# Arbol-Project/dcdf

Measured on NVIDIA B200. Metric: encode_raw_input_GBps, higher is better.
Workload: dtype i64

## Files before the change

### dcdf_b200/csrc/api_encode.cu

```cuda
#include <algorithm>
#include <chrono>
#include <cmath>
#include <cstdlib>
#include <mutex>

#include "encode_big.cuh"
#include "encode_v4.cuh"
#include "encode_v5.cuh"
#include "gather.cuh"
#include "host.hpp"
#include "tree_geo.hpp"
#include "stats.cuh"
#include "xfer.cuh"

using namespace dcdf;

namespace dcdf {
void free_chunk_meta(void* p);
void free_super_meta(void* p);
}

namespace {

int32_t status_from_flags(u32 f, std::string& msg) {
  if (f & EF_NONFINITE) { msg = "cannot convert a non-finite value to fixed point (fixed.rs:39-41)"; return DCDF_ERR_NONFINITE; }
  if (f & EF_OVERFLOW) { msg = "overflow converting to fixed point (fixed.rs:66-69)"; return DCDF_ERR_OVERFLOW; }
  if (f & EF_PRECISION) { msg = "loss of precision converting to fixed point (fixed.rs:51-57)"; return DCDF_ERR_PRECISION_LOSS; }
  if (f & EF_BAD_LEVELS) { msg = "tree levels passed in do not match the levels a nested sub-array needs (superchunk.rs:105-110)"; return DCDF_ERR_BAD_LEVELS; }
  if (f & EF_REGION_EXACT) { msg = "nested region with negatives far below its positive range needs the exact fraction pass, which is not built for nested superchunks yet"; return DCDF_ERR_BAD_ARG; }
  if (f & EF_BAD_FORMAT) { msg = "internal consistency check failed in the encoder"; return DCDF_ERR_BAD_FORMAT; }
  if (f & EF_OUT_CAP) { msg = "output buffer too small"; return DCDF_ERR_BAD_ARG; }
  return DCDF_OK;
}

size_t elem_size(int enc) { return (enc == DCDF_ENC_I32 || enc == DCDF_ENC_F32) ? 4 : 8; }

template <typename Fn>
int32_t guarded(dcdf_ctx* ctx, Fn&& fn) {
  if (!ctx) return DCDF_ERR_BAD_ARG;
  try {
    cudaError_t e = cudaSetDevice(ctx->device);
    if (e != cudaSuccess) throw CudaFail{std::string("cudaSetDevice: ") + cudaGetErrorString(e)};
    fn();
    return DCDF_OK;
  } catch (const ApiFail& f) {
    ctx->last_error = f.msg;
    return f.code;
  } catch (const CudaFail& f) {
    ctx->last_error = f.msg;
    cudaGetLastError();
    return DCDF_ERR_CUDA;
  } catch (const std::bad_alloc&) {
    ctx->last_error = "host out of memory";
    return DCDF_ERR_BAD_ARG;
  } catch (const std::exception& e) {
    ctx->last_error = std::string("unexpected exception: ") + e.what();
    return DCDF_ERR_BAD_ARG;
  } catch (...) {
    ctx->last_error = "unexpected exception";
    return DCDF_ERR_BAD_ARG;
  }
}

void validate_array(const dcdf_array3* a) {
  if (!a || !a->base) api_fail(DCDF_ERR_BAD_ARG, "null array");
  if (a->encoding != DCDF_ENC_I32 && a->encoding != DCDF_ENC_I64 && a->encoding != DCDF_ENC_F32 && a->encoding != DCDF_ENC_F64)
    api_fail(DCDF_ERR_BAD_ARG, "bad encoding %d", a->encoding);
  for (int i = 0; i < 3; i++) {
    if (a->shape[i] <= 0) api_fail(DCDF_ERR_BAD_ARG, "empty array axis %d", i);
  }
  if (a->mem != DCDF_MEM_HOST && a->mem != DCDF_MEM_DEVICE) api_fail(DCDF_ERR_BAD_ARG, "bad mem kind");
}

const void* stage_input(dcdf_ctx* ctx, const dcdf_array3* a) {
  if (a->mem == DCDF_MEM_DEVICE) return a->base;
  int64_t lo = 0, hi = 0;
  for (int i = 0; i < 3; i++) {
    const int64_t ext = (a->shape[i] - 1) * a->strides[i];
    if (ext < 0) lo += ext; else hi += ext;
  }
  const size_t es = elem_size(a->encoding);
  const size_t bytes = (size_t)(hi - lo + 1) * es;
  ctx->input_copy.reserve(bytes);
  static std::mutex upload_mutex[64];
  std::lock_guard<std::mutex> lock(upload_mutex[ctx->device & 63]);
  CK(cudaMemcpyAsync(ctx->input_copy.p, static_cast<const char*>(a->base) + lo * (int64_t)es, bytes, cudaMemcpyHostToDevice, ctx->stream));
  CK(cudaStreamSynchronize(ctx->stream));
  return static_cast<const char*>(ctx->input_copy.p) - lo * (int64_t)es;
}

struct EncodeJob {
  const void* dev_data = nullptr;
  int encoding = 0;
  int64_t strides[3] = {0, 0, 0};
  std::vector<EncUnit> units;
  std::vector<SliceDesc> slices;
  std::vector<uint64_t> table_len;
  uint32_t n_slots = 1;
  uint32_t t_max = 1;
  int plain = 0, req_bits = 0, round = 0, compute_bits = 0;
  int64_t rows = 0, cols = 0;
  size_t input_bytes = 0;
  TreeGeo* tree = nullptr;
};

struct EncodeOut {
  std::vector<EncUnit> units;
  std::vector<UnitResult> results;
  std::vector<uint8_t> stored;
  std::vector<uint64_t> chunk_off;
  std::vector<SliceState> states;
  std::vector<Piece> dac_pieces;
  std::vector<Piece> pieces;
  uint8_t* blob = nullptr;
  uint64_t blob_size = 0;
  uint8_t* dac_blob = nullptr;
  uint64_t dac_blob_size = 0;
  std::vector<uint64_t> dac_off;
  std::vector<NodeState> nstate;
  int64_t* tbl_max = nullptr;
  int64_t* tbl_min = nullptr;
  uint64_t tbl_total = 0;
};

template <typename InT, typename V, bool FULL, int MINB>
void launch_encode_one(dcdf_ctx* ctx, const EncParams& P, u32 grid) {
  const size_t smem = sizeof(EncSmem<V>);
  CK(cudaFuncSetAttribute(k_encode_tiles<InT, V, FULL, MINB>, cudaFuncAttributeMaxDynamicSharedMemorySize, (int)smem));
  k_encode_tiles<InT, V, FULL, MINB><<<grid, ENC_THREADS, smem, FULL ? ctx->stream : ctx->aux_stream>>>(P);
  CK(cudaGetLastError());
  ctx->launches++;
}
template <typename InT, bool FULL>
void launch_encode_v4(dcdf_ctx* ctx, const EncParams& P, u32 grid) {
  constexpr int MINB = 4;
  const u32 stage_limit = std::min<u32>(ctx->opt.stage_limit, (u32)E4_POOL);
  const size_t smem = sizeof(E4Smem);
  CK(cudaFuncSetAttribute(k_encode_v4<InT, MINB, FULL>, cudaFuncAttributeMaxDynamicSharedMemorySize, (int)smem));
  k_encode_v4<InT, MINB, FULL><<<grid, E4_THREADS, smem, FULL ? ctx->stream : ctx->aux_stream>>>(P, stage_limit);
  CK(cudaGetLastError());
  ctx->launches++;
}
template <int G, bool BULK>
void launch_encode_v5_variant(dcdf_ctx* ctx, const EncParams& P, u32 grid) {
  const u32 stage_limit = std::min<u32>(ctx->opt.stage_limit, (u32)E5_POOL);
  const size_t smem = (sizeof(E5Smem) + (BULK ? sizeof(E5Bulk) : 0)) * G;
  CK(cudaFuncSetAttribute(k_encode_v5<G, true, BULK>, cudaFuncAttributeMaxDynamicSharedMemorySize, (int)smem));
  k_encode_v5<G, true, BULK><<<(grid + G - 1) / G, E5_THREADS * G, smem, ctx->stream>>>(P, stage_limit, ctx->opt.fast_sync_mask);
  CK(cudaGetLastError());
  ctx->launches++;
}
template <bool FULL>
void launch_encode_v5(dcdf_ctx* ctx, const EncParams& P, u32 grid) {
  constexpr int G = 6;
  if (FULL && ctx->opt.fast_variant == 1) return launch_encode_v5_variant<4, false>(ctx, P, grid);
  if (FULL && ctx->opt.fast_variant == 2 && ((P.stride_r | P.stride_t) & 3) == 0 && (((uintptr_t)P.data + 4 * 0) & 15) == 0)
    return launch_encode_v5_variant<4, true>(ctx, P, grid);
  const u32 stage_limit = std::min<u32>(ctx->opt.stage_limit, (u32)E5_POOL);
  const size_t smem = sizeof(E5Smem) * G;
  CK(cudaFuncSetAttribute(k_encode_v5<G, FULL>, cudaFuncAttributeMaxDynamicSharedMemorySize, (int)smem));
  k_encode_v5<G, FULL><<<(grid + G - 1) / G, E5_THREADS * G, smem, FULL ? ctx->stream : ctx->aux_stream>>>(P, stage_limit, ctx->opt.fast_sync_mask);
  CK(cudaGetLastError());
  ctx->launches++;
}
void launch_encode_v5_edge(dcdf_ctx* ctx, const EncParams& P, u32 grid) {
  constexpr int G = 12;
  const u32 stage_limit = std::min<u32>(ctx->opt.stage_limit, (u32)E5_POOL_EDGE);
  const size_t smem = sizeof(E5SmemEdge) * G;
  CK(cudaFuncSetAttribute(k_encode_v5_edge<G>, cudaFuncAttributeMaxDynamicSharedMemorySize, (int)smem));
  k_encode_v5_edge<G><<<(grid + G - 1) / G, 32 * G, smem, ctx->aux_stream>>>(P, stage_limit, ctx->opt.fast_sync_mask);
  CK(cudaGetLastError());
  ctx->launches++;
}
template <typename InT>
void launch_encode(dcdf_ctx* ctx, const EncParams& P, u32 grid, int list) {
  if (grid == 0) return;
  if (list >= 5) {
    if (sizeof(InT) == 4) {
      if (list == 5) launch_encode_v5<true>(ctx, P, grid);
      else if (list == 6) launch_encode_v5<false>(ctx, P, grid);
      else launch_encode_v5_edge(ctx, P, grid);
    }
    return;
  }
  const bool force_v2 = ctx->opt.encode_tiles256 != 0;
  if (list == 0 && !force_v2) { launch_encode_v4<InT, true>(ctx, P, grid); return; }
  if (list == 4 && !force_v2) { launch_encode_v4<InT, false>(ctx, P, grid); return; }
  switch (list) {
    case 0: launch_encode_one<InT, int32_t, true, 2>(ctx, P, grid); break;
    case 1: case 4: launch_encode_one<InT, int32_t, false, 2>(ctx, P, grid); break;
    case 2: launch_encode_one<InT, i64, true, 1>(ctx, P, grid); break;
    default: launch_encode_one<InT, i64, false, 1>(ctx, P, grid); break;
  }
}

template <typename InT, bool IS_FLOAT>
void launch_stats(dcdf_ctx* ctx, const StatParams& P) {
  k_unit_stats<InT, IS_FLOAT><<<P.n_units, STAT_THREADS, 0, ctx->stream>>>(P);
  CK(cudaGetLastError());
  ctx->launches++;
}

void time_begin(dcdf_ctx* ctx, int which) { CK(cudaEventRecord(ctx->ev[2 * which], ctx->stream)); }
void time_end(dcdf_ctx* ctx, int which) { CK(cudaEventRecord(ctx->ev[2 * which + 1], ctx->stream)); }
void time_collect(dcdf_ctx* ctx, int which) {
  float ms = 0;
  if (cudaEventElapsedTime(&ms, ctx->ev[2 * which], ctx->ev[2 * which + 1]) == cudaSuccess) ctx->kernel_ms[which] = ms;
  else cudaGetLastError();
}

struct Tracer {
  bool on;
  cudaStream_t st;
  std::chrono::steady_clock::time_point t0;
  Tracer(cudaStream_t s, bool on_) : on(on_), st(s), t0(std::chrono::steady_clock::now()) {}
  void mark(const char* what) {
    if (!on) return;
    cudaStreamSynchronize(st);
    auto t1 = std::chrono::steady_clock::now();
    fprintf(stderr, "[dcdf trace] %-28s %9.3f ms\n", what, std::chrono::duration<double, std::milli>(t1 - t0).count());
    t0 = t1;
  }
};

void run_encode(dcdf_ctx* ctx, EncodeJob& job, EncodeOut& out, bool want_pieces) {
  cudaStream_t st = ctx->stream;
  Tracer tr(st, ctx->opt.trace != 0);
  const u32 n_units = (u32)job.units.size();
  const u32 n_slices = (u32)job.slices.size();
  if (n_units == 0) api_fail(DCDF_ERR_BAD_ARG, "nothing to encode");
  u64 n_pieces = 0;
  for (auto& u : job.units) { u.piece_base = (u32)n_pieces; n_pieces += (u64)u.instants; }
  if (n_pieces > 0xfffffff0ull) api_fail(DCDF_ERR_BAD_ARG, "too many (unit, instant) pairs for one call");
  u64 tbl_total = 0;
  const u32 n_nodes = job.tree ? (u32)job.tree->nodes.size() : 1u;
  const u32 n_tables = n_slices * n_nodes;
  std::vector<uint64_t> table_base(n_tables), table_len(n_tables);
  for (u32 s = 0; s < n_slices; s++) {
    job.slices[s].table_base = tbl_total;
    for (u32 n = 0; n < n_nodes; n++) {
      const u64 off = job.tree ? (u64)job.tree->nodes[n].tbl_off : 0, nch = job.tree ? (u64)job.tree->nodes[n].n_children : 0;
      table_base[(size_t)s * n_nodes + n] = tbl_total + off * (u64)job.slices[s].instants;
      table_len[(size_t)s * n_nodes + n] = job.plain ? 0 : nch * (u64)job.slices[s].instants;
    }
    tbl_total += job.plain ? 0 : job.table_len[s];
  }

  ctx->units.reserve(sizeof(EncUnit) * n_units);
  ctx->ustats.reserve(sizeof(UnitStats) * n_units);
  ctx->istats.reserve(sizeof(InstStats) * (size_t)n_units * job.t_max);
  ctx->slices.reserve(sizeof(SliceDesc) * n_slices + 2 * sizeof(u64) * n_tables);
  ctx->sstate.reserve(sizeof(SliceState) * n_slices);
  ctx->order.reserve(sizeof(u32) * (8 * (size_t)n_units + 8));
  ctx->pieces.reserve(sizeof(Piece) * (n_pieces + 2 * (size_t)n_tables));
  ctx->results.reserve(sizeof(UnitResult) * n_units);
  ctx->stored.reserve(n_units);
  ctx->chunk_off.reserve(sizeof(u64) * ((size_t)n_units + 1));
  ctx->small.reserve(256);
  if (!job.plain) ctx->tbl_scratch.reserve(sizeof(u64) * 4 * tbl_total);
  int64_t *d_tbl_max = nullptr, *d_tbl_min = nullptr;
  if (!job.plain && tbl_total) {
    d_tbl_max = static_cast<int64_t*>(pool_alloc(sizeof(i64) * tbl_total, st));
    d_tbl_min = static_cast<int64_t*>(pool_alloc(sizeof(i64) * tbl_total, st));
  }
  out.tbl_max = d_tbl_max;
  out.tbl_min = d_tbl_min;
  out.tbl_total = tbl_total;

  u32* d_err = ctx->small.as<u32>();
  unsigned long long* d_head = reinterpret_cast<unsigned long long*>(ctx->small.as<u8>() + 8);
  u32* d_counts = reinterpret_cast<u32*>(ctx->small.as<u8>() + 16);

  ctx->pin.reserve(sizeof(EncUnit) * n_units + sizeof(SliceDesc) * n_slices + 2 * sizeof(u64) * n_tables + 64);
  EncUnit* h_units = ctx->pin.as<EncUnit>();
  memcpy(h_units, job.units.data(), sizeof(EncUnit) * n_units);
  SliceDesc* h_slices = reinterpret_cast<SliceDesc*>(h_units + n_units);
  memcpy(h_slices, job.slices.data(), sizeof(SliceDesc) * n_slices);
  u64* h_tb = reinterpret_cast<u64*>(h_slices + n_slices);
  for (u32 i = 0; i < n_tables; i++) { h_tb[i] = table_base[i]; h_tb[n_tables + i] = table_len[i]; }
  copy_by_kernel(ctx, ctx->units.p, h_units, sizeof(EncUnit) * n_units);
  copy_by_kernel(ctx, ctx->slices.p, h_slices, sizeof(SliceDesc) * n_slices + 2 * sizeof(u64) * n_tables);
  const u64* d_table_base = reinterpret_cast<const u64*>(ctx->slices.as<SliceDesc>() + n_slices);
  const u64* d_table_len = d_table_base + n_tables;
  TreeNode* d_nodes = nullptr;
  TreeChild* d_children = nullptr;
  int32_t* d_leaf_unit = nullptr;
  NodeState* d_nstate = nullptr;
  if (job.tree) {
    const TreeGeo& G = *job.tree;
    const size_t b0 = sizeof(TreeNode) * G.nodes.size(), b1 = sizeof(TreeChild) * G.children.size(),
                 b2 = sizeof(int32_t) * G.leaf_unit.size(), b3 = sizeof(NodeState) * (size_t)n_tables;
    ctx->tree_buf.reserve(b0 + b1 + b2 + b3 + 1024);
    u8* tb = ctx->tree_buf.as<u8>();
    d_nodes = reinterpret_cast<TreeNode*>(tb);
    d_children = reinterpret_cast<TreeChild*>(tb + ((b0 + 255) & ~size_t(255)));
    d_leaf_unit = reinterpret_cast<int32_t*>(reinterpret_cast<u8*>(d_children) + ((b1 + 255) & ~size_t(255)));
    d_nstate = reinterpret_cast<NodeState*>(reinterpret_cast<u8*>(d_leaf_unit) + ((b2 + 255) & ~size_t(255)));
    upload_small(ctx, d_nodes, G.nodes.data(), b0);
    upload_small(ctx, d_children, G.children.data(), b1);
    upload_small(ctx, d_leaf_unit, G.leaf_unit.data(), b2);
  }

  tr.mark("scratch + uploads");
  StatParams SP;
  SP.data = job.dev_data;
  SP.stride_t = job.strides[0]; SP.stride_r = job.strides[1]; SP.stride_c = job.strides[2];
  SP.units = ctx->units.as<EncUnit>();
  SP.n_units = n_units;
  SP.t_max = job.t_max;
  SP.ustats = ctx->ustats.as<UnitStats>();
  SP.istats = ctx->istats.as<InstStats>();
  time_begin(ctx, KT_STATS);
  switch (job.encoding) {
    case DCDF_ENC_F32: launch_stats<float, true>(ctx, SP); break;
    case DCDF_ENC_F64: launch_stats<double, true>(ctx, SP); break;
    case DCDF_ENC_I32: launch_stats<int32_t, false>(ctx, SP); break;
    default: launch_stats<i64, false>(ctx, SP); break;
  }
  time_end(ctx, KT_STATS);
  tr.mark("k_unit_stats");

  FinalizeParams FP;
  FP.slices = ctx->slices.as<SliceDesc>();
  FP.state = ctx->sstate.as<SliceState>();
  FP.units_in = ctx->units.as<EncUnit>();
  FP.units = ctx->units.as<EncUnit>();
  FP.ustats = SP.ustats;
  FP.istats = SP.istats;
  FP.t_max = job.t_max;
  FP.n_slots = job.n_slots;
  FP.encoding = job.encoding;
  FP.req_bits = job.req_bits; FP.round = job.round; FP.compute_bits = job.compute_bits; FP.plain = job.plain;
  FP.tbl_min = d_tbl_min; FP.tbl_max = d_tbl_max;
  FP.order = ctx->order.as<u32>();
  FP.order_pitch = n_units;
  FP.order_counts = d_counts;
  FP.stored = ctx->stored.as<u8>();
  FP.err = d_err;
  CK(cudaMemsetAsync(ctx->small.p, 0, 64, st));
  k_finalize_phase1<<<n_slices, 256, 0, st>>>(FP, n_slices);
  CK(cudaGetLastError());
  ctx->launches++;
  const bool is_float = job.encoding == DCDF_ENC_F32 || job.encoding == DCDF_ENC_F64;
  if (is_float && job.compute_bits) {
    SliceState* ss = ctx->sstate.as<SliceState>();
    std::vector<SliceState> hs(n_slices);
    read_small(ctx, hs.data(), ss, sizeof(SliceState) * n_slices);
    sync_reads(ctx);
    bool any = false;
    for (auto& s : hs) any = any || s.need_exact;
    if (any) {
      ctx->exact.reserve((sizeof(i64) + 5 * sizeof(int)) * n_slices + 64);
      std::vector<i64> t0(n_slices);
      std::vector<int> inst(n_slices);
      for (u32 s = 0; s < n_slices; s++) { t0[s] = job.slices[s].t0; inst[s] = job.slices[s].instants; }
      i64* d_t0 = ctx->exact.as<i64>();
      int* d_inst = reinterpret_cast<int*>(d_t0 + n_slices);
      upload_small(ctx, d_t0, t0.data(), sizeof(i64) * n_slices);
      upload_small(ctx, d_inst, inst.data(), sizeof(int) * n_slices);
      ExactParams XP;
      XP.data = job.dev_data;
      XP.stride_t = job.strides[0]; XP.stride_r = job.strides[1]; XP.stride_c = job.strides[2];
      XP.rows = job.rows; XP.cols = job.cols;
      XP.slice_t0 = d_t0; XP.slice_instants = d_inst;
      std::vector<int> need(n_slices), maxfb(n_slices);
      for (u32 s = 0; s < n_slices; s++) { need[s] = hs[s].need_exact; maxfb[s] = hs[s].maxfb; }
      int* d_need = d_inst + n_slices;
      int* d_maxfb = d_need + n_slices;
      int* d_f = d_maxfb + n_slices;
      int* d_round = d_f + n_slices;
      upload_small(ctx, d_need, need.data(), sizeof(int) * n_slices);
      upload_small(ctx, d_maxfb, maxfb.data(), sizeof(int) * n_slices);
      CK(cudaMemsetAsync(d_f, 0, 2 * sizeof(int) * n_slices, st));
      XP.slice_need = d_need; XP.slice_maxfb = d_maxfb; XP.slice_f = d_f; XP.slice_round = d_round;
      dim3 grid((unsigned)std::min<int64_t>(4 * ctx->sm_count, 65535), n_slices);
      if (job.encoding == DCDF_ENC_F32) k_fraction_exact<float><<<grid, 256, 0, st>>>(XP, n_slices);
      else k_fraction_exact<double><<<grid, 256, 0, st>>>(XP, n_slices);
      CK(cudaGetLastError());
      ctx->launches++;
      std::vector<int> f(n_slices), r(n_slices);
      read_small(ctx, f.data(), d_f, sizeof(int) * n_slices);
      read_small(ctx, r.data(), d_round, sizeof(int) * n_slices);
      sync_reads(ctx);
      for (u32 s = 0; s < n_slices; s++) { hs[s].f_exact = f[s]; hs[s].round_exact = r[s]; }
      upload_small(ctx, ss, hs.data(), sizeof(SliceState) * n_slices);
    }
  }
  if (job.tree) {
    const TreeGeo& G = *job.tree;
    TreeParams TP;
    TP.slices = FP.slices; TP.state = FP.state;
    TP.nodes = d_nodes; TP.children = d_children; TP.n_nodes = n_nodes;
    TP.leaf_unit = d_leaf_unit; TP.leaf_cols = G.leaf_cols; TP.leaf_side = G.leaf_side;
    TP.tbl_per_instant = G.tbl_per_instant;
    TP.nstate = d_nstate;
    TP.units = ctx->units.as<EncUnit>();
    TP.ustats = SP.ustats; TP.istats = SP.istats; TP.t_max = job.t_max;
    TP.encoding = job.encoding; TP.round = job.round; TP.req_bits = job.req_bits;
    TP.allow_fast = job.encoding == DCDF_ENC_F32 && !ctx->opt.no_fast_encode && job.strides[2] == 1;
    TP.tbl_min = d_tbl_min; TP.tbl_max = d_tbl_max;
    TP.order = FP.order; TP.order_pitch = FP.order_pitch; TP.order_counts = FP.order_counts;
    TP.stored = FP.stored; TP.err = d_err;
    k_finalize_tree<<<n_slices, 256, 0, st>>>(TP, n_slices);
  } else {
    k_finalize_phase2<<<n_slices, 256, 0, st>>>(FP, n_slices);
  }
  CK(cudaGetLastError());
  ctx->launches++;

  tr.mark("finalize");
  if (ctx->arena_hint == 0) ctx->arena_hint = std::max<size_t>(job.input_bytes / 2 + (8u << 20), 16u << 20);
  std::vector<uint8_t> head_buf(64);
  u32 sticky = 0;
  for (int attempt = 0;; attempt++) {
    ctx->arena.reserve(ctx->arena_hint);
    const u64 arena_cap = ctx->arena.cap;
    CK(cudaMemsetAsync(d_head, 0, 8, st));
    EncParams EP;
    EP.data = job.dev_data;
    EP.stride_t = job.strides[0]; EP.stride_r = job.strides[1]; EP.stride_c = job.strides[2];
    EP.units = ctx->units.as<EncUnit>();
    EP.pieces = ctx->pieces.as<Piece>();
    EP.results = ctx->results.as<UnitResult>();
    EP.arena = ctx->arena.as<u8>();
    EP.arena_cap = arena_cap;
    EP.arena_head = d_head;
    EP.err = d_err;
    time_begin(ctx, KT_ENCODE);
    CK(cudaEventRecord(ctx->fork_ev, st));
    CK(cudaStreamWaitEvent(ctx->aux_stream, ctx->fork_ev, 0));
    for (int list = 7; list >= 0; list--) {
      EP.order = FP.order + (size_t)list * n_units;
      EP.order_count = d_counts + list;
      switch (job.encoding) {
        case DCDF_ENC_F32: launch_encode<float>(ctx, EP, n_units, list); break;
        case DCDF_ENC_F64: launch_encode<double>(ctx, EP, n_units, list); break;
        case DCDF_ENC_I32: launch_encode<int32_t>(ctx, EP, n_units, list); break;
        default: launch_encode<i64>(ctx, EP, n_units, list); break;
      }
    }
    CK(cudaEventRecord(ctx->join_ev, ctx->aux_stream));
    CK(cudaStreamWaitEvent(st, ctx->join_ev, 0));
    time_end(ctx, KT_ENCODE);
    tr.mark("k_encode_tiles");
    if (!job.plain) {
      TableDacParams TP;
      TP.tbl_min = d_tbl_min; TP.tbl_max = d_tbl_max;
      TP.table_base = d_table_base; TP.table_len = d_table_len;
      TP.alive = reinterpret_cast<const int*>(d_nstate);
      TP.scratch = ctx->tbl_scratch.as<u64>();
      TP.total = tbl_total;
      TP.pieces = ctx->pieces.as<Piece>() + n_pieces;
      TP.arena = ctx->arena.as<u8>(); TP.arena_cap = arena_cap; TP.arena_head = d_head; TP.err = d_err;
      k_table_dac<<<dim3(n_tables, 2), ENC_THREADS, 0, st>>>(TP);
      CK(cudaGetLastError());
      ctx->launches++;
    }
    tr.mark("k_table_dac");
    k_scan_units<<<1, 1024, 0, st>>>(ctx->results.as<UnitResult>(), ctx->stored.as<u8>(), n_units, ctx->chunk_off.as<u64>());
    CK(cudaGetLastError());
    ctx->launches++;
    read_small(ctx, head_buf.data(), ctx->small.p, 64);
    sync_reads(ctx);
    u32 flags;
    u64 head;
    memcpy(&flags, head_buf.data(), 4);
    memcpy(&head, head_buf.data() + 8, 8);
    memcpy(ctx->last_list_counts, head_buf.data() + 16, sizeof ctx->last_list_counts);
    sticky |= flags & ~(u32)EF_ARENA_FULL;
    std::string msg;
    if ((flags & EF_ARENA_FULL) && status_from_flags(sticky, msg) == DCDF_OK) {
      if (attempt >= 3) api_fail(DCDF_ERR_CUDA, "arena overflow persisted after growth");
      ctx->arena_hint = (size_t)head + (size_t)head / 16 + (1u << 20);
      CK(cudaMemsetAsync(d_err, 0, 4, st));
      continue;
    }
    flags = sticky;
    int32_t code = status_from_flags(flags, msg);
    if (code != DCDF_OK) {
      pool_free(d_tbl_max);
      pool_free(d_tbl_min);
      out.tbl_max = out.tbl_min = nullptr;
      throw ApiFail{code, msg};
    }
    break;
  }
  time_collect(ctx, KT_STATS);
  time_collect(ctx, KT_ENCODE);
  tr.mark("scan + flags readback");

  out.units.resize(n_units);
  out.results.resize(n_units);
  out.stored.resize(n_units);
  out.chunk_off.resize((size_t)n_units + 1);
  out.states.resize(n_slices);
  read_small(ctx, out.units.data(), ctx->units.p, sizeof(EncUnit) * n_units);
  read_small(ctx, out.results.data(), ctx->results.p, sizeof(UnitResult) * n_units);
  read_small(ctx, out.stored.data(), ctx->stored.p, n_units);
  read_small(ctx, out.chunk_off.data(), ctx->chunk_off.p, sizeof(u64) * ((size_t)n_units + 1));
  read_small(ctx, out.states.data(), ctx->sstate.p, sizeof(SliceState) * n_slices);
  if (!job.plain) {
    out.dac_pieces.resize(2 * (size_t)n_tables);
    read_small(ctx, out.dac_pieces.data(), ctx->pieces.as<Piece>() + n_pieces, sizeof(Piece) * 2 * n_tables);
    out.nstate.resize(n_tables);
    read_small(ctx, out.nstate.data(), d_nstate, sizeof(NodeState) * n_tables);
  }
  if (want_pieces) {
    out.pieces.resize(n_pieces);
    CK(cudaMemcpyAsync(out.pieces.data(), ctx->pieces.p, sizeof(Piece) * n_pieces, cudaMemcpyDeviceToHost, st));
  }
  sync_reads(ctx);

  tr.mark("tables readback");
  out.blob_size = out.chunk_off[n_units];
  out.blob = static_cast<uint8_t*>(pool_alloc(out.blob_size + 64, st));
  CK(cudaMemsetAsync(out.blob + out.blob_size, 0, 64, st));
  GatherParams GP;
  GP.units = ctx->units.as<EncUnit>();
  GP.results = ctx->results.as<UnitResult>();
  GP.stored = ctx->stored.as<u8>();
  GP.pieces = ctx->pieces.as<Piece>();
  GP.chunk_off = ctx->chunk_off.as<u64>();
  GP.arena = ctx->arena.as<u8>();
  GP.out = out.blob;
  GP.out_cap = out.blob_size;
  GP.encoding = job.encoding;
  GP.n_units = n_units;
  GP.err = d_err;
  tr.mark("blob alloc");
  time_begin(ctx, KT_GATHER);
  k_gather_chunks<<<n_units, 256, 0, st>>>(GP);
  CK(cudaGetLastError());
  ctx->launches++;
  if (!job.plain) {
    out.dac_off.resize(2 * (size_t)n_tables);
    u64 off = 0;
    for (u32 i = 0; i < 2 * n_tables; i++) { out.dac_off[i] = off; off += out.dac_pieces[i].size; }
    out.dac_blob_size = off;
    out.dac_blob = static_cast<uint8_t*>(pool_alloc(off + 16, st));
    ctx->query_aux.reserve(sizeof(u64) * 2 * n_tables);
    upload_small(ctx, ctx->query_aux.p, out.dac_off.data(), sizeof(u64) * 2 * n_tables);
    GatherDacParams DP;
    DP.pieces = ctx->pieces.as<Piece>() + n_pieces;
    DP.dst_off = ctx->query_aux.as<u64>();
    DP.arena = ctx->arena.as<u8>();
    DP.out = out.dac_blob;
    k_gather_dacs<<<2 * n_tables, 256, 0, st>>>(DP);
    CK(cudaGetLastError());
    ctx->launches++;
  }
  time_end(ctx, KT_GATHER);
  read_small(ctx, head_buf.data(), ctx->small.p, 4);
  sync_reads(ctx);
  time_collect(ctx, KT_GATHER);
  tr.mark("gather");
  u32 flags;
  memcpy(&flags, head_buf.data(), 4);
  flags |= sticky;
  std::string msg;
  int32_t code = status_from_flags(flags, msg);
  if (code != DCDF_OK) throw ApiFail{code, msg};
}


struct BigResult {
  uint8_t* blob = nullptr;
  uint64_t size = 0;
  uint32_t snapshots = 0, logs = 0;
  std::vector<uint32_t> block_instants;
};

struct BigScratch {
  dcdf_ctx* ctx;
  u8* base = nullptr;
  size_t used = 0, cap = 0;
  template <typename T>
  T* take(size_t n) {
    used = (used + 255) & ~size_t(255);
    T* p = reinterpret_cast<T*>(base + used);
    used += n * sizeof(T);
    return p;
  }
};

unsigned big_grid(dcdf_ctx* ctx, u64 n, int block = 256) {
  return (unsigned)std::max<u64>(1, std::min<u64>((n + block - 1) / block, (u64)ctx->sm_count * 16));
}

void big_scan(dcdf_ctx* ctx, const u64* in, u64 n, u64* out, u64* block_sums) {
  if (n == 0) return;
  const unsigned nb = (unsigned)((n + SCAN_ITEMS - 1) / SCAN_ITEMS);
// ... 828 lines not shown
```

### dcdf_b200/csrc/encode_v5.cuh

```cuda
#pragma once
#include <type_traits>

#include "encode_v4.cuh"

namespace dcdf {

constexpr int E5_THREADS = 64;
constexpr int E5_POOL = 9 * 1024;
constexpr int E5_POOL_EDGE = 5 * 1024;

template <int TT, int POOL>
struct E5SmemT {
  __align__(16) u8 pool[POOL + 16];
  int4 cell[16][TT];
  int2 l4s[4][TT];
  int2 l4t[4][TT];
  u32 leaf[16][TT];
  u32 qx[4][TT];
  u32 qn[4][TT];
  int4 rec1[4];
  int2 ent1[4];
  u32 wt[2][2][4];
  u32 bm_off[12], bm_len[12];
  u32 n_bm;
// ... 101 lines not shown
    if (t.len > 3) b3[p3] = (u8)(t.z >> 24);
  }
}
template <bool FULL>
DCDF_DEVINL void e5_load_node(const float* pn, i64 sr, uint4 (&raw)[4], int rl, int cl, int vec) {
#pragma unroll
  for (int r = 0; r < 4; r++) {
    if (FULL || (r < rl && cl >= 4)) {
      const float* pr = pn + (i64)r * sr;
      if (vec == 2) {
        asm volatile("ld.shared.v4.u32 {%0, %1, %2, %3}, [%4];" : "=r"(raw[r].x), "=r"(raw[r].y), "=r"(raw[r].z), "=r"(raw[r].w)
                     : "r"((u32)__cvta_generic_to_shared(pr)));
      } else if (vec) {
        raw[r] = __ldg(reinterpret_cast<const uint4*>(pr));
      } else {
        raw[r] = make_uint4(__float_as_uint(__ldg(pr)), __float_as_uint(__ldg(pr + 1)), __float_as_uint(__ldg(pr + 2)), __float_as_uint(__ldg(pr + 3)));
      }
    } else {
      raw[r] = make_uint4(0, 0, 0, 0);
      if (r < rl) {
        const float* pr = pn + (i64)r * sr;
        if (cl > 0) raw[r].x = __float_as_uint(__ldg(pr));
        if (cl > 1) raw[r].y = __float_as_uint(__ldg(pr + 1));
        if (cl > 2) raw[r].z = __float_as_uint(__ldg(pr + 2));
      }
    }
  }
}
DCDF_DEVINL int e5_conv_raw(float x, float scale2) { return __float_as_int(__fmaf_rn(x, scale2, 12582912.0f)) - (0x4B400000 - 1); }
DCDF_DEVINL int e5_nan0(u32 bits, int f) { return (bits & 0x7fffffffu) > 0x7f800000u ? 0 : f; }
template <bool FULL>
DCDF_DEVINL void e5_quads(const uint4 (&raw)[4], float scale2, int4 (&q)[4], int rl, int cl) {
#pragma unroll
  for (int h = 0; h < 2; h++) {
    const uint4 u = raw[2 * h], l = raw[2 * h + 1];
    q[2 * h] = make_int4(e5_conv_raw(__uint_as_float(u.x), scale2), e5_conv_raw(__uint_as_float(u.y), scale2),
                         e5_conv_raw(__uint_as_float(l.x), scale2), e5_conv_raw(__uint_as_float(l.y), scale2));
    q[2 * h + 1] = make_int4(e5_conv_raw(__uint_as_float(u.z), scale2), e5_conv_raw(__uint_as_float(u.w), scale2),
                             e5_conv_raw(__uint_as_float(l.z), scale2), e5_conv_raw(__uint_as_float(l.w), scale2));
  }
  {
    const int m01 = max(max(max(q[0].x, q[0].y), max(q[0].z, q[0].w)), max(max(q[1].x, q[1].y), max(q[1].z, q[1].w)));
    const int m23 = max(max(max(q[2].x, q[2].y), max(q[2].z, q[2].w)), max(max(q[3].x, q[3].y), max(q[3].z, q[3].w)));
    if (max(m01, m23) > (1 << 28)) {
#pragma unroll
      for (int h = 0; h < 2; h++) {
        const uint4 u = raw[2 * h], l = raw[2 * h + 1];
        q[2 * h] = make_int4(e5_nan0(u.x, q[2 * h].x), e5_nan0(u.y, q[2 * h].y), e5_nan0(l.x, q[2 * h].z), e5_nan0(l.y, q[2 * h].w));
        q[2 * h + 1] = make_int4(e5_nan0(u.z, q[2 * h + 1].x), e5_nan0(u.w, q[2 * h + 1].y), e5_nan0(l.z, q[2 * h + 1].z), e5_nan0(l.w, q[2 * h + 1].w));
      }
    }
  }
#pragma unroll
  for (int h = 0; h < 2; h++) {
    if (!FULL) {
      const bool ru = 2 * h < rl, rw = 2 * h + 1 < rl;
      if (!(ru && cl > 0)) q[2 * h].x = E4_NONE;
      if (!(ru && cl > 1)) q[2 * h].y = E4_NONE;
      if (!(rw && cl > 0)) q[2 * h].z = E4_NONE;
      if (!(rw && cl > 1)) q[2 * h].w = E4_NONE;
      if (!(ru && cl > 2)) q[2 * h + 1].x = E4_NONE;
      if (!(ru && cl > 3)) q[2 * h + 1].y = E4_NONE;
      if (!(rw && cl > 2)) q[2 * h + 1].z = E4_NONE;
      if (!(rw && cl > 3)) q[2 * h + 1].w = E4_NONE;
    }
  }
}
DCDF_DEVINL const float* e5_node_ptr(const float* pt, i64 sr, int a) { return pt + (i64)(4 * (a >> 1)) * sr + 4 * (a & 1); }
template <bool FULL>
DCDF_DEVINL int e5_dx(int a, int b) { return e4_sub(e4_o0<FULL>(a), e4_o0<FULL>(b)); }
DCDF_DEVINL int e5_dn(int a, int b) { return e4_sub(a, b); }

DCDF_DEVINL u32 e5_low4(int a, int b, int c, int d) { return __byte_perm(__byte_perm((u32)a, (u32)b, 0x0040), __byte_perm((u32)c, (u32)d, 0x0040), 0x5410); }
DCDF_DEVINL u32 e5_zz4(u32 p) { return ((p + p) & 0xfefefefeu) ^ (((p >> 7) & 0x01010101u) * 0xffu); }
DCDF_DEVINL u32 e5_pack4(u32 z0, u32 z1, u32 z2, u32 z3) { return (z0 & 0xffu) | ((z1 & 0xffu) << 8) | ((z2 & 0xffu) << 16) | (z3 << 24); }
template <bool ALIGNED = false>
DCDF_DEVINL void e5_store_word(u8* p, u32 w) {
  if (ALIGNED || (((uintptr_t)p) & 3u) == 0) *reinterpret_cast<u32*>(p) = w;
  else { p[0] = (u8)w; p[1] = (u8)(w >> 8); p[2] = (u8)(w >> 16); p[3] = (u8)(w >> 24); }
}

template <bool FULL, int TT = E5_THREADS>
__device__ __noinline__ void e5_long_node(bool as_snapshot, const float* pn, i64 sr, float scale2, const int4* scell, int2 n4, u32 in5a,
                                          u8* xb1, u8* nb1, u32* pos , int rl, int cl, int vec) {
  int4 q[4];
  if (!as_snapshot) {
    uint4 raw[4];
    e5_load_node<FULL>(pn, sr, raw, rl, cl, vec);
    e5_quads<FULL>(raw, scale2, q, rl, cl);
  }
  u32 lx1 = pos[0], rx1 = pos[1], rn1 = pos[2];
  u32 zx[4], zn[4];
#pragma unroll
  for (int b = 0; b < 4; b++) {
    const int4 s = scell[b * TT];
    const int4 t = as_snapshot ? s : q[b];
    int qmax, qmin, sqmax, sqmin;
    e4_qmm<FULL>(t, qmax, qmin);
    e4_qmm<FULL>(s, sqmax, sqmin);
    zx[b] = zigzag32(as_snapshot ? e5_dx<FULL>(n4.x, qmax) : e5_dx<FULL>(qmax, sqmax));
    zn[b] = zigzag32(as_snapshot ? e5_dn(qmin, n4.y) : e5_dn(qmin, sqmin));
    if ((in5a >> (3 - b)) & 1u) {
      const u32 z0 = zigzag32(as_snapshot ? e5_dx<FULL>(qmax, t.x) : e4_sub(t.x, s.x)), z1 = zigzag32(as_snapshot ? e5_dx<FULL>(qmax, t.y) : e4_sub(t.y, s.y));
      const u32 z2 = zigzag32(as_snapshot ? e5_dx<FULL>(qmax, t.z) : e4_sub(t.z, s.z)), z3 = zigzag32(as_snapshot ? e5_dx<FULL>(qmax, t.w) : e4_sub(t.w, s.w));
      if (z0 > 0xffu) xb1[lx1++] = (u8)(z0 >> 8);
      if (z1 > 0xffu) xb1[lx1++] = (u8)(z1 >> 8);
      if (z2 > 0xffu) xb1[lx1++] = (u8)(z2 >> 8);
      if (z3 > 0xffu) xb1[lx1++] = (u8)(z3 >> 8);
    }
  }
#pragma unroll
  for (int b = 0; b < 4; b++)
    if (zx[b] > 0xffu) xb1[rx1++] = (u8)(zx[b] >> 8);
#pragma unroll
  for (int b = 0; b < 4; b++)
    if (((in5a >> (3 - b)) & 1u) && zn[b] > 0xffu) nb1[rn1++] = (u8)(zn[b] >> 8);
  pos[0] = lx1; pos[1] = rx1; pos[2] = rn1;
}

DCDF_DEVINL u32 e5_smem_u32(const void* p) { return (u32)__cvta_generic_to_shared(p); }
DCDF_DEVINL void e5_mbar_init(unsigned long long* b, u32 count) {
  asm volatile("mbarrier.init.shared::cta.b64 [%0], %1;" ::"r"(e5_smem_u32(b)), "r"(count) : "memory");
}
DCDF_DEVINL void e5_mbar_expect_tx(unsigned long long* b, u32 bytes) {
  asm volatile("mbarrier.arrive.expect_tx.shared::cta.b64 _, [%0], %1;" ::"r"(e5_smem_u32(b)), "r"(bytes) : "memory");
}
DCDF_DEVINL void e5_mbar_wait(unsigned long long* b, u32 parity) {
  asm volatile(
      "{\n\t.reg .pred P1;\n\t"
      "E5_WAIT:\n\t"
      "mbarrier.try_wait.parity.shared::cta.b64 P1, [%0], %1;\n\t"
      "@P1 bra E5_DONE;\n\t"
      "bra E5_WAIT;\n\t"
      "E5_DONE:\n\t}" ::"r"(e5_smem_u32(b)), "r"(parity) : "memory");
}
DCDF_DEVINL void e5_bulk_g2s(void* smem, const void* g, u32 bytes, unsigned long long* b) {
  asm volatile("cp.async.bulk.shared::cluster.global.mbarrier::complete_tx::bytes [%0], [%1], %2, [%3];" ::"r"(e5_smem_u32(smem)),
               "l"(g), "r"(bytes), "r"(e5_smem_u32(b))
               : "memory");
}
struct E5Bulk {
  __align__(16) float raw[64 * 64];
  __align__(8) unsigned long long mbar;
  unsigned long long pad_;
};

template <int NW>
DCDF_DEVINL void e5_tile_sync(int slot) {
  if (NW == 1) __syncwarp();
  else asm volatile("bar.sync %0, 64;" ::"r"(slot + 1) : "memory");
}

template <int G, bool FULL, bool BULK, int NW = 2>
DCDF_DEVINL void e5_body(const EncParams& P, const u32 stage_limit, const int sync_mask);
template <int G, bool FULL, bool BULK = false>
__global__ void __launch_bounds__(E5_THREADS * G, 1) k_encode_v5(const EncParams P, const u32 stage_limit, const int sync_mask) {
  e5_body<G, FULL, BULK>(P, stage_limit, sync_mask);
}
template <int G>
__global__ void __launch_bounds__(32 * G, 1) k_encode_v5_edge(const EncParams P, const u32 stage_limit, const int sync_mask) {
  e5_body<G, false, false, 1>(P, stage_limit, sync_mask);
}
template <int G, bool FULL, bool BULK, int NW>
DCDF_DEVINL void e5_body(const EncParams& P, const u32 stage_limit, const int sync_mask) {
  static_assert(NW == 2 || (NW == 1 && !FULL && !BULK), "one-warp tiles are clipped edge tiles");
  constexpr int TT = 32 * NW;
  using Smem = std::conditional_t<NW == 2, E5Smem, E5SmemEdge>;
  const int vec = BULK ? 2 : (((P.stride_r | P.stride_t) & 3) == 0 && (((uintptr_t)P.data) & 15) == 0) ? 1 : 0;
  extern __shared__ __align__(16) unsigned char smem_raw[];
  const int slot = threadIdx.x / TT;
  constexpr size_t kSlab = sizeof(Smem) + (BULK ? sizeof(E5Bulk) : 0);
  Smem& S = *reinterpret_cast<Smem*>(smem_raw + (size_t)slot * kSlab);
  E5Bulk& SB = *reinterpret_cast<E5Bulk*>(smem_raw + (size_t)slot * kSlab + sizeof(Smem));

  const u32 n_order = *P.order_count;
  if (blockIdx.x * (u32)G >= n_order) return;
  const u32 order_idx = blockIdx.x * (u32)G + (u32)slot;
  const bool tile_live = order_idx < n_order;
  const u32 unit_idx = P.order[tile_live ? order_idx : blockIdx.x * (u32)G];
  EncUnit unit = P.units[unit_idx];
  if (!tile_live) unit.instants = 0;
  int max_instants = 0;
  for (int g = 0; g < G; g++) {
    const u32 oi = blockIdx.x * (u32)G + (u32)g;
    if (oi < n_order) max_instants = max(max_instants, P.units[P.order[oi]].instants);
  }
  const int tid = threadIdx.x % TT, lane = tid & 31, warp = tid >> 5;
  const int node = NW == 2 ? tid : unit.rows <= 32 ? lane : lane < 16 ? lane : lane + 16;
  const float scale2 = (float)((i64)2 << unit.bits);
  const i64 sr = BULK ? 64 : P.stride_r;
  const float* const base = BULK ? SB.raw + (8 * (int)morton_row(tid)) * 64 + 8 * (int)morton_col(tid)
                                 : static_cast<const float*>(P.data) + unit.base + (i64)(8 * (int)morton_row(node)) * sr + 8 * (int)morton_col(node);
  const float* const my_row = static_cast<const float*>(P.data) + unit.base + (i64)tid * P.stride_r;
  auto fetch_instant = [&](int t) {
    if (tid == 0) e5_mbar_expect_tx(&SB.mbar, 64u * 256u);
    e5_bulk_g2s(SB.raw + 64 * tid, my_row + (i64)t * P.stride_t, 256u, &SB.mbar);
  };
  if (BULK) {
    if (tid == 0) {
      e5_mbar_init(&SB.mbar, 1u);
      asm volatile("fence.mbarrier_init.release.cluster;" ::: "memory");
    }
    e5_tile_sync<NW>(slot);
    if (unit.instants > 0) fetch_instant(0);
  }
  const bool owner2 = (lane & 3) == 0;
  const bool is1 = (u32)(lane - 1) < 4u;
  const int k1 = node >> 4;
  const int rl8 = unit.rows - 8 * (int)morton_row(node), cl8 = unit.cols - 8 * (int)morton_col(node);
#define E5_RL(a) (rl8 - 4 * ((a) >> 1))
#define E5_CL(a) (cl8 - 4 * ((a) & 1))

  {
    uint4* z = reinterpret_cast<uint4*>(S.pool);
    for (int i = tid; i < (int)(sizeof(S.pool) / 16); i += TT) z[i] = make_uint4(0, 0, 0, 0);
  }
  if (!FULL) {
    for (int q = 0; q < 16; q++) S.cell[q][tid] = make_int4(E4_NONE, E4_NONE, E4_NONE, E4_NONE);
    for (int a = 0; a < 4; a++) S.l4s[a][tid] = make_int2(E4_NONE, INT32_MAX);
  }
  if (NW == 1 && lane == 0) {
    const u32 missing1 = unit.rows <= 32 ? 0xcu : 0xau;
    for (int k = 0; k < 4; k++) {
      if ((missing1 >> k) & 1u) {
        S.rec1[k] = make_int4(E4_NONE, INT32_MAX, 0, 1);
        S.ent1[k] = make_int2(0, 0);
      }
    }
    for (int c = 0; c < 2; c++)
      for (int i = 0; i < 4; i++) S.wt[1][c][i] = 0u;
  }

  u32 err = 0;
  int s3max = 0, s3min = 0, s2max = 0, s2min = 0, s1max = 0, s1min = 0, s0max = 0, s0min = 0;
  u32 n_logs = 0, n_snap = 0, n_log_total = 0;
  u64 total_bytes = 0;

#pragma unroll 1
  for (int inst = 0; inst < max_instants; inst++) {
    if ((inst & sync_mask) == 0) __syncthreads();
    if (inst >= unit.instants) continue;
    const bool first = inst == 0;
    const float* const pt = BULK ? base : base + (i64)inst * P.stride_t;
    if (BULK) e5_mbar_wait(&SB.mbar, (u32)inst & 1u);
    if (!BULK && inst + 1 < unit.instants) {
#pragma unroll
      for (int r = 0; r < 8; r++)
        if (FULL || (r < rl8 && cl8 > 0)) asm volatile("prefetch.global.L2 [%0];" ::"l"(pt + P.stride_t + (i64)r * sr));
    }
    const bool forced = first || n_logs == 254u;

    u32 u5 = 0, eq5 = 0, u4 = 0, eq4 = 0;
    E5Cand L, C;
    L.ml = 0; L.mq = 0; L.mu = 0; L.in5 = 0; L.in4 = 0; L.in3 = L.in2 = L.in1 = false;
    C.ml = 0; C.mq = 0; C.mu = 0; C.in5 = 0; C.in4 = 0; C.in3 = C.in2 = C.in1 = false;
    int t3max = 0, t3min = 0, diff3 = 0;
    bool eq3 = false, u3 = false;
    int t2max = 0, t2min = 0, t1max = 0, t1min = 0, t0max = 0, t0min = 0;
    bool u2 = false, eq2 = false, u0 = false, eq0 = false;
    int n1max = 0, n1min = 0, l_e1max = 0, l_e1min = 0;
    bool n1un = false, n1eq = false;
    u32 l_in1 = 0, s_in1 = 0;
    bool l_in0 = false, s_in0 = false;
    u32 wl[4] = {0, 0, 0, 0}, ws[4] = {0, 0, 0, 0};
    E5Tot T;
    u32 ntop = 0, item_cnt = 0, item_size = 0;
    bool as_snapshot = forced;
    u32 my_size = 0, log_size = 0;

#pragma unroll 1
    for (int pass = forced ? 1 : 0; pass < 2; pass++) {
      t3max = INT32_MIN; t3min = INT32_MAX;
      u5 = 0; u4 = 0;
      uint4 raw[4];
      e5_load_node<FULL>(e5_node_ptr(pt, sr, 0), sr, raw, E5_RL(0), E5_CL(0), vec);
      if (pass == 0) {
        eq3 = true;
#pragma unroll 1
        for (int a = 0; a < 4; a++) {
          int4 q[4];
          e5_quads<FULL>(raw, scale2, q, E5_RL(a), E5_CL(a));
          if (a < 3) e5_load_node<FULL>(e5_node_ptr(pt, sr, a + 1), sr, raw, E5_RL(a + 1), E5_CL(a + 1), vec);
          const int2 s4 = S.l4s[a][tid];
          int amax = INT32_MIN, amin = INT32_MAX, dfirst = 0;
          bool aeq = true;
          u32 leaf16 = 0, u5n = 0, e5n = 0, qx = 0, qn = 0;
          u32 exw = 0, enw = 0;
          u32 ovx = 0, ovn = 0, ovm = 0;
#pragma unroll
          for (int b = 0; b < 4; b++) {
            const int4 t = q[b], sq = S.cell[4 * a + b][tid];
            int qmax, qmin, sqmax, sqmin;
            e4_qmm<FULL>(t, qmax, qmin);
            e4_qmm<FULL>(sq, sqmax, sqmin);
            const int d0 = e4_sub(t.x, sq.x), d1 = e4_sub(t.y, sq.y), d2 = e4_sub(t.z, sq.z), d3 = e4_sub(t.w, sq.w);
            const int ex = e5_dx<FULL>(qmax, sqmax), en = e5_dn(qmin, sqmin);
            const bool e5 = (((d1 ^ d0) | (d2 ^ d0) | (d3 ^ d0)) == 0);
            if (e4_unif<FULL>(qmax, qmin)) u5n |= 1u << (3 - b);
            if (e5) e5n |= 1u << (3 - b);
            u32 leafw = e5_zz4(e5_low4(d0, d1, d2, d3));
            exw = __byte_perm(exw, (u32)ex, b == 0 ? 0x3214 : b == 1 ? 0x3240 : b == 2 ? 0x3410 : 0x4210);
            enw = __byte_perm(enw, (u32)en, b == 0 ? 0x3214 : b == 1 ? 0x3240 : b == 2 ? 0x3410 : 0x4210);
            if ((((u32)d0 + 128u) | ((u32)d1 + 128u) | ((u32)d2 + 128u) | ((u32)d3 + 128u) | ((u32)ex + 128u) | ((u32)en + 128u)) > 255u) {
              if (e4_longer<1>(d0)) leaf16 |= 1u << (15 - 4 * b);
              if (e4_longer<1>(d1)) leaf16 |= 1u << (14 - 4 * b);
              if (e4_longer<1>(d2)) leaf16 |= 1u << (13 - 4 * b);
              if (e4_longer<1>(d3)) leaf16 |= 1u << (12 - 4 * b);
              if (e4_longer<1>(ex)) qx |= 1u << (3 - b);
              if (e4_longer<1>(en)) qn |= 1u << (3 - b);
              if ((((u32)d0 + 32768u) | ((u32)d1 + 32768u) | ((u32)d2 + 32768u) | ((u32)d3 + 32768u)) > 65535u) err |= EF_BAD_FORMAT;
              leafw = e5_pack4(zigzag32(d0), zigzag32(d1), zigzag32(d2), zigzag32(d3));
              ovx |= (zigzag32(ex) & 0xffu) << (8 * b);
              ovn |= (zigzag32(en) & 0xffu) << (8 * b);
              ovm |= 0xffu << (8 * b);
            }
            S.leaf[4 * a + b][tid] = leafw;
            amax = max(amax, qmax); amin = min(amin, qmin);
            if (b == 0) dfirst = d0;
            aeq = aeq && e5 && d0 == dfirst;
          }
          const u32 zxw = (e5_zz4(exw) & ~ovm) | ovx, znw = (e5_zz4(enw) & ~ovm) | ovn;
          S.qx[a][tid] = zxw;
          S.qn[a][tid] = znw;
          S.l4t[a][tid] = make_int2(amax, amin);
          L.ml |= (u64)leaf16 << (48 - 16 * a);
          L.mq |= (qx << (12 - 4 * a)) | (qn << (28 - 4 * a));
          u5 |= u5n << (12 - 4 * a);
          eq5 |= e5n << (12 - 4 * a);
          if (e4_unif<FULL>(amax, amin)) u4 |= 1u << (3 - a);
          if (aeq) eq4 |= 1u << (3 - a);
          if (e4_longer<1>(e5_dx<FULL>(amax, s4.x))) L.mu |= 1u << (3 - a);
          if (e4_longer<1>(e5_dn(amin, s4.y))) L.mu |= 1u << (7 - a);
          t3max = max(t3max, amax); t3min = min(t3min, amin);
          if (a == 0) diff3 = dfirst;
          eq3 = eq3 && aeq && dfirst == diff3;
        }
        if (e4_longer<1>(e5_dx<FULL>(t3max, s3max))) L.mu |= 1u << 8;
// ... 369 lines not shown
      }
    }
    if (emit) {
      if (x4) {
        u32 rx1 = bx4 + e4_f4(pre[1]), rn1 = bn4 + e4_f4(pre[3]);
        u32 zx[4], zn[4];
#pragma unroll
        for (int a = 0; a < 4; a++) {
          const int2 n4 = S.l4t[a][tid];
          const int2 s4 = as_snapshot ? make_int2(0, 0) : S.l4s[a][tid];
          zx[a] = zigzag32(as_snapshot ? e5_dx<FULL>(t3max, n4.x) : e5_dx<FULL>(n4.x, s4.x));
          zn[a] = zigzag32(as_snapshot ? e5_dn(n4.y, t3min) : e5_dn(n4.y, s4.y));
        }
        e5_store_word<decltype(in_shared)::value>(xb0 + Pn4 + 4u * R3, e5_pack4(zx[0], zx[1], zx[2], zx[3]));
        u8* dmn = nb0 + Mn4 + R4;
        if (W.mu & 0xffu) {
#pragma unroll
          for (int a = 0; a < 4; a++)
            if (zx[a] > 0xffu) rx1 = e5_hi(xb1, zx[a], rx1);
        }
#pragma unroll
        for (int a = 0; a < 4; a++) {
          if ((W.in4 >> (3 - a)) & 1u) {
            *dmn++ = (u8)zn[a];
            if (zn[a] > 0xffu) rn1 = e5_hi(nb1, zn[a], rn1);
          }
        }
      }
      if (x3) {
        const u32 zx = zigzag32(as_snapshot ? e5_dx<FULL>(t2max, t3max) : e5_dx<FULL>(t3max, s3max));
        xb0[Pn3 + 4u * R2p + (u32)(node & 3)] = (u8)zx;
        if (zx > 0xffu) e5_hi(xb1, zx, bx3 + e4_f3(pre[1]));
        if (W.in3) {
          const u32 zn = zigzag32(as_snapshot ? e5_dn(t3min, t2min) : e5_dn(t3min, s3min));
          nb0[Mn3 + R3] = (u8)zn;
          if (zn > 0xffu) e5_hi(nb1, zn, bn3 + e4_f3(pre[3]));
        }
      }
      if (x2 && owner2) {
        const u32 zx = zigzag32(as_snapshot ? e5_dx<FULL>(t1max, t2max) : e5_dx<FULL>(t2max, s2max));
        xb0[Pn2 + 4u * R1 + (u32)((node >> 2) & 3)] = (u8)zx;
        if (zx > 0xffu) e5_hi(xb1, zx, bx2 + e4_f2(pre[1]));
        if (W.in2) {
          const u32 zn = zigzag32(as_snapshot ? e5_dn(t2min, t1min) : e5_dn(t2min, s2min));
          nb0[Mn2 + R2own] = (u8)zn;
          if (zn > 0xffu) e5_hi(nb1, zn, bn2 + e4_f2(pre[3]));
        }
      }
#pragma unroll
      for (int r = 0; r < NTOP; r++) {
        const bool mx = NW == 2 ? warp == 0 : r == 0;
        if (top[r].len > 0) (mx ? xb0 : nb0)[top[r].pos0] = (u8)top[r].z;
        if (top[r].len > 1) (mx ? xb1 : nb1)[top[r].pos1] = (u8)(top[r].z >> 8);
        if (__any_sync(0xffffffffu, top[r].len > 2)) e5_top_long(true, out, top[r], mx ? 2 : 6, item_hdr, item_cnt, item_at);
      }
      if ((NW == 1 || warp == 1) && lane >= 16) {
        const u32 i = lane - 16u;
        if (i < 13u) {
          const u32 word = i < 5u ? (u32)unit.rows : i < 9u ? (u32)unit.cols : 64u;
          out[i] = i == 0 ? (u8)2 : (u8)(word >> (8u * ((12u - i) & 3u)));
        } else if (i == 13u) {
          out[x_hdr0 - 1] = (u8)x_levels;
        } else if (i == 14u) {
          out[n_hdr0 - 1] = (u8)n_levels;
        }
      }
    }
    e5_tile_sync<NW>(slot);
    if (BULK && inst + 1 < unit.instants) fetch_instant(inst + 1);

    if (emit) {
      const u32 n_fix = as_snapshot ? 1u : 2u;
      const u32 n_bm = n_fix + x_levels + n_levels;
#pragma unroll 1
      for (u32 i = warp; i < n_bm; i += NW) {
        const int src = (int)(i < n_fix ? i : i < n_fix + x_levels ? 2u + (i - n_fix) : 6u + (i - n_fix - x_levels));
        const u32 hdr = shfl(item_hdr, src), len = shfl(item_cnt, src);
        if (lane == 0) {
          store_be32(out + hdr, len);
          store_be32(out + hdr + 4, 4u);
        }
        const u32 blocks = len >> 7;
        u8* const index = out + hdr + 8u;
        const u8* const words = index + 4u * blocks;
        u32 carry = 0;
#pragma unroll 1
        for (u32 b0 = 0; b0 < blocks; b0 += 32u) {
          const u32 b = b0 + lane;
          u32 c = b < blocks ? e4_popc_bytes16(words + 16u * b) : 0u;
#pragma unroll
          for (int d = 1; d < 32; d <<= 1) {
            const u32 n = __shfl_up_sync(0xffffffffu, c, d);
            if (lane >= d) c += n;
          }
          if (b < blocks) e4_store_be32(index + 4u * b, carry + c);
          carry += shfl(c, 31);
        }
      }
    }
    if (decltype(in_shared)::value && tid == 0) publish_piece();
    e5_tile_sync<NW>(slot);

    if constexpr (decltype(in_shared)::value) {
      piece_off = S.piece_off;
      fits = piece_off + (((u64)my_size + 15ull) & ~15ull) <= P.arena_cap;
      if (!fits) err |= EF_ARENA_FULL;
      u32* src = reinterpret_cast<u32*>(S.pool);
      uint4* dst = reinterpret_cast<uint4*>(P.arena + piece_off);
      const u32 sh = 8u * shift;
      const u32 n16 = (my_size + 15u) / 16u;
#pragma unroll 1
      for (u32 i = tid; i < n16; i += TT) {
        const uint4 v = *reinterpret_cast<const uint4*>(src + 4u * i);
        const u32 nx = src[4u * i + 4u];
        uint4 o;
        o.x = __funnelshift_r(v.x, v.y, sh); o.y = __funnelshift_r(v.y, v.z, sh);
        o.z = __funnelshift_r(v.z, v.w, sh); o.w = __funnelshift_r(v.w, nx, sh);
        if (fits) dst[i] = o;
      }
      e5_tile_sync<NW>(slot);
#pragma unroll 1
      for (u32 i = tid; i < n16 + 1u; i += TT) *reinterpret_cast<uint4*>(src + 4u * i) = make_uint4(0, 0, 0, 0);
    }

    };
    if (staged) emission(std::true_type{});
    else emission(std::false_type{});

    if (as_snapshot) {
      s3max = t3max; s3min = t3min; s2max = t2max; s2min = t2min; s1max = t1max; s1min = t1min; s0max = t0max; s0min = t0min;
      n_snap++;
      n_logs = 0;
      total_bytes += 1;
    } else {
      n_logs++;
      n_log_total++;
    }
    total_bytes += my_size;
  }

  if (tid == 0 && tile_live) {
    UnitResult r;
    r.bytes = total_bytes + 6;
    r.snapshots = n_snap;
    r.logs = n_log_total;
    P.results[unit_idx] = r;
  }
  err = __reduce_or_sync(0xffffffffu, err);
  if (lane == 0 && err) atomicOr(P.err, err);
#undef E5_RL
#undef E5_CL
}

}
```

Baseline: 663.1.

## Merge full and edge tile encoders into one persistent work-stealing kernel

After: 654.3 (median of 6 runs). 0.987x the previous value.

```diff
diff --git a/dcdf_b200/csrc/api_encode.cu b/dcdf_b200/csrc/api_encode.cu
--- a/dcdf_b200/csrc/api_encode.cu
+++ b/dcdf_b200/csrc/api_encode.cu
@@ -153,9 +153,6 @@
 template <bool FULL>
 void launch_encode_v5(dcdf_ctx* ctx, const EncParams& P, u32 grid) {
   constexpr int G = 6;
-  if (FULL && ctx->opt.fast_variant == 1) return launch_encode_v5_variant<4, false>(ctx, P, grid);
-  if (FULL && ctx->opt.fast_variant == 2 && ((P.stride_r | P.stride_t) & 3) == 0 && (((uintptr_t)P.data + 4 * 0) & 15) == 0)
-    return launch_encode_v5_variant<4, true>(ctx, P, grid);
   const u32 stage_limit = std::min<u32>(ctx->opt.stage_limit, (u32)E5_POOL);
   const size_t smem = sizeof(E5Smem) * G;
   CK(cudaFuncSetAttribute(k_encode_v5<G, FULL>, cudaFuncAttributeMaxDynamicSharedMemorySize, (int)smem));
@@ -163,23 +160,29 @@
   CK(cudaGetLastError());
   ctx->launches++;
 }
-void launch_encode_v5_edge(dcdf_ctx* ctx, const EncParams& P, u32 grid) {
-  constexpr int G = 12;
-  const u32 stage_limit = std::min<u32>(ctx->opt.stage_limit, (u32)E5_POOL_EDGE);
-  const size_t smem = sizeof(E5SmemEdge) * G;
-  CK(cudaFuncSetAttribute(k_encode_v5_edge<G>, cudaFuncAttributeMaxDynamicSharedMemorySize, (int)smem));
-  k_encode_v5_edge<G><<<(grid + G - 1) / G, 32 * G, smem, ctx->aux_stream>>>(P, stage_limit, ctx->opt.fast_sync_mask);
+void launch_encode_v5_sched(dcdf_ctx* ctx, const EncParams& P, u32 n_units, E5Sched Q) {
+  Q.stage_full = std::min<u32>(ctx->opt.stage_limit, (u32)E5_POOL);
+  Q.stage_edge = std::min<u32>(ctx->opt.stage_limit, (u32)E5_POOL_EDGE);
+  Q.with_full = 1;
+  if (ctx->opt.fast_variant == 1) { launch_encode_v5_variant<4, false>(ctx, P, n_units); Q.with_full = 0; }
+  if (ctx->opt.fast_variant == 2 && ((P.stride_r | P.stride_t) & 3) == 0 && (((uintptr_t)P.data) & 15) == 0) {
+    launch_encode_v5_variant<4, true>(ctx, P, n_units);
+    Q.with_full = 0;
+  }
+  const u32 groups = (n_units + E5_GE - 1) / E5_GE + (Q.with_full ? (n_units + E5_GF - 1) / E5_GF : 0u);
+  const u32 grid = std::min<u32>((u32)ctx->sm_count, groups);
+  CK(cudaFuncSetAttribute(k_encode_v5_sched, cudaFuncAttributeMaxDynamicSharedMemorySize, (int)E5_SCHED_SMEM));
+  k_encode_v5_sched<<<grid, E5_SCHED_THREADS, E5_SCHED_SMEM, ctx->stream>>>(P, Q, ctx->opt.fast_sync_mask);
   CK(cudaGetLastError());
   ctx->launches++;
 }
 template <typename InT>
-void launch_encode(dcdf_ctx* ctx, const EncParams& P, u32 grid, int list) {
+void launch_encode(dcdf_ctx* ctx, const EncParams& P, u32 grid, int list, const E5Sched& Q) {
   if (grid == 0) return;
   if (list >= 5) {
     if (sizeof(InT) == 4) {
-      if (list == 5) launch_encode_v5<true>(ctx, P, grid);
+      if (list == 5) launch_encode_v5_sched(ctx, P, grid, Q);
       else if (list == 6) launch_encode_v5<false>(ctx, P, grid);
-      else launch_encode_v5_edge(ctx, P, grid);
     }
     return;
   }
@@ -270,6 +273,7 @@
   u32* d_err = ctx->small.as<u32>();
   unsigned long long* d_head = reinterpret_cast<unsigned long long*>(ctx->small.as<u8>() + 8);
   u32* d_counts = reinterpret_cast<u32*>(ctx->small.as<u8>() + 16);
+  u32* d_next = reinterpret_cast<u32*>(ctx->small.as<u8>() + 48);
 
   ctx->pin.reserve(sizeof(EncUnit) * n_units + sizeof(SliceDesc) * n_slices + 2 * sizeof(u64) * n_tables + 64);
   EncUnit* h_units = ctx->pin.as<EncUnit>();
@@ -416,6 +420,7 @@
     ctx->arena.reserve(ctx->arena_hint);
     const u64 arena_cap = ctx->arena.cap;
     CK(cudaMemsetAsync(d_head, 0, 8, st));
+    CK(cudaMemsetAsync(d_next, 0, 4, st));
     EncParams EP;
     EP.data = job.dev_data;
     EP.stride_t = job.strides[0]; EP.stride_r = job.strides[1]; EP.stride_c = job.strides[2];
@@ -426,6 +431,10 @@
     EP.arena_cap = arena_cap;
     EP.arena_head = d_head;
     EP.err = d_err;
+    E5Sched EQ{};
+    EQ.order_edge = FP.order + (size_t)7 * n_units;
+    EQ.count_edge = d_counts + 7;
+    EQ.next = d_next;
     time_begin(ctx, KT_ENCODE);
     CK(cudaEventRecord(ctx->fork_ev, st));
     CK(cudaStreamWaitEvent(ctx->aux_stream, ctx->fork_ev, 0));
@@ -433,10 +442,10 @@
       EP.order = FP.order + (size_t)list * n_units;
       EP.order_count = d_counts + list;
       switch (job.encoding) {
-        case DCDF_ENC_F32: launch_encode<float>(ctx, EP, n_units, list); break;
-        case DCDF_ENC_F64: launch_encode<double>(ctx, EP, n_units, list); break;
-        case DCDF_ENC_I32: launch_encode<int32_t>(ctx, EP, n_units, list); break;
-        default: launch_encode<i64>(ctx, EP, n_units, list); break;
+        case DCDF_ENC_F32: launch_encode<float>(ctx, EP, n_units, list, EQ); break;
+        case DCDF_ENC_F64: launch_encode<double>(ctx, EP, n_units, list, EQ); break;
+        case DCDF_ENC_I32: launch_encode<int32_t>(ctx, EP, n_units, list, EQ); break;
+        default: launch_encode<i64>(ctx, EP, n_units, list, EQ); break;
       }
     }
     CK(cudaEventRecord(ctx->join_ev, ctx->aux_stream));
diff --git a/dcdf_b200/csrc/encode_v5.cuh b/dcdf_b200/csrc/encode_v5.cuh
--- a/dcdf_b200/csrc/encode_v5.cuh
+++ b/dcdf_b200/csrc/encode_v5.cuh
@@ -277,17 +277,13 @@
 }
 
 template <int G, bool FULL, bool BULK, int NW = 2>
-DCDF_DEVINL void e5_body(const EncParams& P, const u32 stage_limit, const int sync_mask);
+DCDF_DEVINL void e5_body(const EncParams& P, const u32 stage_limit, const int sync_mask, const u32 group);
 template <int G, bool FULL, bool BULK = false>
 __global__ void __launch_bounds__(E5_THREADS * G, 1) k_encode_v5(const EncParams P, const u32 stage_limit, const int sync_mask) {
-  e5_body<G, FULL, BULK>(P, stage_limit, sync_mask);
-}
-template <int G>
-__global__ void __launch_bounds__(32 * G, 1) k_encode_v5_edge(const EncParams P, const u32 stage_limit, const int sync_mask) {
-  e5_body<G, false, false, 1>(P, stage_limit, sync_mask);
+  e5_body<G, FULL, BULK>(P, stage_limit, sync_mask, blockIdx.x);
 }
 template <int G, bool FULL, bool BULK, int NW>
-DCDF_DEVINL void e5_body(const EncParams& P, const u32 stage_limit, const int sync_mask) {
+DCDF_DEVINL void e5_body(const EncParams& P, const u32 stage_limit, const int sync_mask, const u32 group) {
   static_assert(NW == 2 || (NW == 1 && !FULL && !BULK), "one-warp tiles are clipped edge tiles");
   constexpr int TT = 32 * NW;
   using Smem = std::conditional_t<NW == 2, E5Smem, E5SmemEdge>;
@@ -299,15 +295,15 @@
   E5Bulk& SB = *reinterpret_cast<E5Bulk*>(smem_raw + (size_t)slot * kSlab + sizeof(Smem));
 
   const u32 n_order = *P.order_count;
-  if (blockIdx.x * (u32)G >= n_order) return;
-  const u32 order_idx = blockIdx.x * (u32)G + (u32)slot;
+  if (group * (u32)G >= n_order) return;
+  const u32 order_idx = group * (u32)G + (u32)slot;
   const bool tile_live = order_idx < n_order;
-  const u32 unit_idx = P.order[tile_live ? order_idx : blockIdx.x * (u32)G];
+  const u32 unit_idx = P.order[tile_live ? order_idx : group * (u32)G];
   EncUnit unit = P.units[unit_idx];
   if (!tile_live) unit.instants = 0;
   int max_instants = 0;
   for (int g = 0; g < G; g++) {
-    const u32 oi = blockIdx.x * (u32)G + (u32)g;
+    const u32 oi = group * (u32)G + (u32)g;
     if (oi < n_order) max_instants = max(max_instants, P.units[P.order[oi]].instants);
   }
   const int tid = threadIdx.x % TT, lane = tid & 31, warp = tid >> 5;
@@ -983,4 +979,37 @@
 #undef E5_CL
 }
 
-}
+constexpr int E5_GF = 6, E5_GE = 12;
+constexpr int E5_SCHED_THREADS = E5_THREADS * E5_GF;
+static_assert(32 * E5_GE == E5_SCHED_THREADS, "both kinds of group fill the CTA");
+constexpr size_t E5_SCHED_SMEM = sizeof(E5Smem) * E5_GF > sizeof(E5SmemEdge) * E5_GE ? sizeof(E5Smem) * E5_GF : sizeof(E5SmemEdge) * E5_GE;
+struct E5Sched {
+  const u32* order_edge;
+  const u32* count_edge;
+  u32 stage_full, stage_edge;
+  u32 with_full;
+  u32* next;
+};
+__global__ void __launch_bounds__(E5_SCHED_THREADS, 1) k_encode_v5_sched(const EncParams P, const E5Sched Q, const int sync_mask) {
+  __shared__ u32 s_group;
+  const u32 n_edge = (*Q.count_edge + E5_GE - 1) / E5_GE;
+  const u32 n_groups = n_edge + (Q.with_full ? (*P.order_count + E5_GF - 1) / E5_GF : 0u);
+  auto next_group = [&]() {
+    __syncthreads();
+    if (threadIdx.x == 0) s_group = atomicAdd(Q.next, 1u);
+    __syncthreads();
+    return s_group;
+  };
+  u32 g = next_group();
+  if (g < n_edge) {
+    EncParams E = P;
+    E.order = Q.order_edge;
+    E.order_count = Q.count_edge;
+#pragma unroll 1
+    for (; g < n_edge; g = next_group()) e5_body<E5_GE, false, false, 1>(E, Q.stage_edge, sync_mask, g);
+  }
+#pragma unroll 1
+  for (; g < n_groups; g = next_group()) e5_body<E5_GF, true, false, 2>(P, Q.stage_full, sync_mask, g - n_edge);
+}
+
+}
```
